# microsoft/crescent-credentials

Hardware: AMD Instinct MI355X
Metric: Groth16 proofs/sec (rs256-sd-shaped circuit, BN254), G1 MSM scalar-adds/sec reported alongside (higher is better)
Workload: dtype u32 limbs (BN254 Fq/Fr, 254-bit modular integers)

## Files before the change

### crescent-credentials_amd/csrc/csr_host.hpp

```cpp
#pragma once
#include <string.h>

#include <algorithm>
#include <unordered_map>
#include <vector>

#include "curve.hpp"
#include "errors.hpp"
#include "host_parallel.hpp"

namespace cg {

static constexpr uint32_t SELL_PIECE = 8;
static constexpr uint32_t SELL_FINAL = 0x80000000u;
static constexpr uint32_t SELL_PAD = 0xffffffffu;

struct HostSellLevel {
    uint32_t n_pieces = 0, n_partials = 0;
    std::vector<uint32_t> slice_ptr;
    RawArray<uint32_t> dst, col, cidx;
    size_t n_slots = 0;
};
struct HostCsr {
    uint64_t rows = 0, nnz = 0;
    std::vector<uint32_t> rp;
    RawArray<uint32_t> idx;
    std::vector<Fr> dict_mont;
    std::vector<uint32_t> long_rows;
    std::vector<HostSellLevel> levels;
    uint32_t sell_scratch = 0;
};

inline std::vector<uint64_t> range_bounds(uint64_t n, uint64_t min_chunk) {
    uint64_t parts = std::min<uint64_t>(host_threads(), (n + min_chunk - 1) / (min_chunk ? min_chunk : 1));
    if (parts < 1) parts = 1;
    std::vector<uint64_t> b(parts + 1);
    for (uint64_t k = 0; k <= parts; ++k) b[k] = n * k / parts;
    return b;
}
template <class Fn>
inline void for_ranges(const std::vector<uint64_t>& bounds, Fn fn) {
    const uint64_t parts = bounds.size() - 1;
    parallel_ranges(parts, 1, [&](uint64_t a, uint64_t b) { for (uint64_t k = a; k < b; ++k) fn(k, bounds[k], bounds[k + 1]); });
}

#ifdef CSR_HOST_TIMING
#include <chrono>
#include <stdio.h>
#define CSR_LAP(name) do { auto _n = std::chrono::steady_clock::now(); fprintf(stderr, "    %-28s %.1f ms\n", name, std::chrono::duration<double, std::milli>(_n - _lap).count()); _lap = _n; } while (0)
#define CSR_LAP_START auto _lap = std::chrono::steady_clock::now()
#else
#define CSR_LAP(name) do {} while (0)
#define CSR_LAP_START do {} while (0)
#endif
namespace csr_detail {
struct Key {
    uint64_t w[4];
    bool operator==(const Key& o) const { return !memcmp(w, o.w, 32); }
};
struct KeyHash {
    size_t operator()(const Key& k) const { return (size_t)(k.w[0] * 0x9e3779b97f4a7c15ull ^ k.w[1] ^ (k.w[2] << 1) ^ (k.w[3] << 7)); }
};
}

inline void csr_build_sell_host(HostCsr& out, const uint32_t* col_h, bool reorder);

inline void csr_prepare_host(const cg_csr& m, uint64_t rows, uint64_t num_variables, bool sliced, bool reorder, HostCsr& out) {
    using namespace csr_detail;
    out.rows = rows;
    out.nnz = m.nnz;
    const uint64_t nnz = m.nnz;
    if (nnz >= (1ull << 32)) throw HipError(CG_ERR_INVALID_ARGUMENT, "matrix with >= 2^32 non-zeros");
    if (m.row_ptr[0] != 0 || m.row_ptr[rows] != nnz) throw HipError(CG_ERR_INVALID_ARGUMENT, "row_ptr does not span [0, nnz]");
    CSR_LAP_START;
    out.rp.resize(rows + 1);
    parallel_ranges(rows + 1, 1u << 16, [&](uint64_t lo, uint64_t hi) {
        for (uint64_t i = lo; i < hi; ++i) {
            if (i && m.row_ptr[i] < m.row_ptr[i - 1]) throw HipError(CG_ERR_INVALID_ARGUMENT, "row_ptr not monotone");
            out.rp[i] = (uint32_t)m.row_ptr[i];
        }
    });
    CSR_LAP("row_ptr");
    out.idx.alloc(nnz);
    uint32_t* idx = out.idx.p;
    const std::vector<uint64_t> tb = range_bounds(nnz, 1u << 16);
    const uint64_t parts = tb.size() - 1;
    std::vector<std::vector<Key>> local_keys(parts);
    for (auto& v : local_keys) v.reserve(1024);
    for_ranges(tb, [&](uint64_t k, uint64_t lo, uint64_t hi) {
        std::unordered_map<Key, uint32_t, KeyHash> map;
        std::vector<Key>& keys = local_keys[k];
        Key last{};
        uint32_t last_id = 0;
        bool have_last = false;
        for (uint64_t t = lo; t < hi; ++t) {
            if (m.col[t] >= num_variables) throw HipError(CG_ERR_INVALID_ARGUMENT, "column index out of range");
            Key key;
            memcpy(key.w, m.coeff + 32 * t, 32);
            if (key.w[0] == 1 && !(key.w[1] | key.w[2] | key.w[3])) { idx[t] = 0; continue; }
            if (have_last && key == last) { idx[t] = last_id; continue; }
            auto it = map.find(key);
            if (it == map.end()) {
                it = map.emplace(key, (uint32_t)keys.size()).first;
                keys.push_back(key);
            }
            last = key; last_id = it->second | 0x80000000u; have_last = true;
            idx[t] = last_id;
        }
    });
    CSR_LAP("local dictionaries");
    std::vector<Fr> dict_h;
    {
        Fr o = Fr::zero(); o.l[0] = 1;
        dict_h.push_back(o);
    }
    constexpr uint32_t MERGE_PARTS = 16;
    std::vector<std::vector<uint32_t>> remap(parts);
    for (uint64_t k = 0; k < parts; ++k) remap[k].resize(local_keys[k].size());
    std::vector<std::vector<Key>> class_keys(MERGE_PARTS);
    std::vector<std::exception_ptr> class_err(MERGE_PARTS);
    parallel_ranges(MERGE_PARTS, 1, [&](uint64_t lo, uint64_t hi) {
        for (uint64_t cls = lo; cls < hi; ++cls) {
            std::unordered_map<Key, uint32_t, KeyHash> mine;
            std::vector<Key>& ck = class_keys[cls];
            for (uint64_t k = 0; k < parts; ++k)
                for (size_t j = 0; j < local_keys[k].size(); ++j) {
                    const Key& key = local_keys[k][j];
                    if ((KeyHash()(key) >> 7) % MERGE_PARTS != cls) continue;
                    auto it = mine.find(key);
                    if (it == mine.end()) {
                        bool lt = false;
                        for (int q = 3; q >= 0; --q) {
                            const uint64_t nq = (uint64_t)FrP::N[2 * q] | ((uint64_t)FrP::N[2 * q + 1] << 32);
                            if (key.w[q] != nq) { lt = key.w[q] < nq; break; }
                        }
                        if (!lt) throw HipError(CG_ERR_INVALID_ARGUMENT, "non-canonical matrix coefficient");
                        it = mine.emplace(key, (uint32_t)ck.size()).first;
                        ck.push_back(key);
                    }
                    remap[k][j] = it->second | ((uint32_t)cls << 27);
                }
        }
    });
    uint32_t class_off[MERGE_PARTS + 1];
    class_off[0] = 1;
    for (uint32_t cls = 0; cls < MERGE_PARTS; ++cls) {
        if (class_keys[cls].size() >= (1u << 27)) throw HipError(CG_ERR_INVALID_ARGUMENT, "too many distinct matrix coefficients");
        class_off[cls + 1] = class_off[cls] + (uint32_t)class_keys[cls].size();
    }
    dict_h.resize(class_off[MERGE_PARTS]);
    parallel_ranges(MERGE_PARTS, 1, [&](uint64_t lo, uint64_t hi) {
        for (uint64_t cls = lo; cls < hi; ++cls)
            for (size_t j = 0; j < class_keys[cls].size(); ++j) memcpy(dict_h[class_off[cls] + j].l, class_keys[cls][j].w, 32);
    });
    for (uint64_t k = 0; k < parts; ++k)
        for (uint32_t& v : remap[k]) v = class_off[v >> 27] + (v & ((1u << 27) - 1));
    CSR_LAP("merge");
    for_ranges(tb, [&](uint64_t k, uint64_t lo, uint64_t hi) {
        const uint32_t* rm = remap[k].data();
        for (uint64_t t = lo; t < hi; ++t)
            if (idx[t] & 0x80000000u) idx[t] = rm[idx[t] & 0x7fffffffu];
    });
    parallel_ranges(dict_h.size(), 1u << 12, [&](uint64_t lo, uint64_t hi) { for (uint64_t i = lo; i < hi; ++i) dict_h[i] = to_mont(dict_h[i]); });
    out.dict_mont.swap(dict_h);
    CSR_LAP("remap + to_mont");
    out.long_rows.clear();
    for (uint64_t i = 0; i < rows; ++i)
        if (out.rp[i + 1] - out.rp[i] > 4096u) out.long_rows.push_back((uint32_t)i);
    out.levels.clear();
    out.sell_scratch = 0;
    CSR_LAP("long rows");
    if (sliced) csr_build_sell_host(out, m.col, reorder);
    CSR_LAP("sliced layout");
}

inline void csr_build_sell_host(HostCsr& out, const uint32_t* col_h, bool reorder) {
    struct Item { uint32_t row, first, len; };
    struct Piece { uint32_t first, len, dst; };
    const uint64_t rows = out.rows, nnz = out.nnz;
    const std::vector<uint32_t>& rp = out.rp;
    CSR_LAP_START;
    RawArray<uint32_t> cur_col, cur_idx;
    cur_col.alloc(nnz);
    cur_idx.alloc(nnz);
    parallel_ranges(nnz, 1u << 18, [&](uint64_t lo, uint64_t hi) {
        memcpy(cur_col.p + lo, col_h + lo, (hi - lo) * 4);
        memcpy(cur_idx.p + lo, out.idx.p + lo, (hi - lo) * 4);
    });
    if (reorder)
        parallel_ranges(rows, 1u << 14, [&](uint64_t lo, uint64_t hi) {
            for (uint64_t i = lo; i < hi; ++i) {
                uint32_t w = rp[i];
                for (uint32_t t = rp[i]; t < rp[i + 1]; ++t)
                    if (cur_idx.p[t] != 0) {
                        std::swap(cur_idx.p[t], cur_idx.p[w]);
                        std::swap(cur_col.p[t], cur_col.p[w]);
                        ++w;
                    }
            }
        });
    CSR_LAP("  copy + reorder");
    RawArray<Item> items;
    size_t n_items = 0;
    {
        const std::vector<uint64_t> rb = range_bounds(rows, 1u << 14);
        std::vector<uint64_t> cnt(rb.size(), 0);
        for_ranges(rb, [&](uint64_t k, uint64_t lo, uint64_t hi) {
            uint64_t c = 0;
            for (uint64_t i = lo; i < hi; ++i) c += rp[i + 1] > rp[i];
            cnt[k + 1] = c;
        });
        for (size_t k = 1; k < cnt.size(); ++k) cnt[k] += cnt[k - 1];
        n_items = cnt.back();
        items.alloc(n_items);
        for_ranges(rb, [&](uint64_t k, uint64_t lo, uint64_t hi) {
            uint64_t at = cnt[k];
            for (uint64_t i = lo; i < hi; ++i)
                if (rp[i + 1] > rp[i]) items.p[at++] = {(uint32_t)i, rp[i], rp[i + 1] - rp[i]};
        });
    }
    CSR_LAP("  items");
    const uint32_t* ccol = cur_col.p;
    const uint32_t* cidx = cur_idx.p;
    RawArray<uint32_t> next_col_buf;
    while (n_items) {
        if (out.levels.size() >= 8) throw HipError(CG_ERR_INVALID_ARGUMENT, "matrix row too long for the sliced layout");
        out.levels.emplace_back();
        HostSellLevel& L = out.levels.back();
        const std::vector<uint64_t> ib = range_bounds(n_items, 1u << 13);
        const size_t nr = ib.size() - 1;
        std::vector<uint64_t> c_pieces(nr + 1, 0), c_next(nr + 1, 0), c_part(nr + 1, 0);
        for_ranges(ib, [&](uint64_t k, uint64_t lo, uint64_t hi) {
            uint64_t p = 0, n = 0, q = 0;
            for (uint64_t i = lo; i < hi; ++i) {
                const uint32_t np = (items.p[i].len + SELL_PIECE - 1) / SELL_PIECE;
                p += np;
                if (np > 1) { n += 1; q += np; }
            }
            c_pieces[k + 1] = p; c_next[k + 1] = n; c_part[k + 1] = q;
        });
        for (size_t k = 1; k <= nr; ++k) { c_pieces[k] += c_pieces[k - 1]; c_next[k] += c_next[k - 1]; c_part[k] += c_part[k - 1]; }
        const uint64_t n_pieces = c_pieces[nr], partials = c_part[nr];
        if (n_pieces >= (1ull << 31) || partials >= (1ull << 31)) throw HipError(CG_ERR_INVALID_ARGUMENT, "matrix too large for the sliced layout");
        RawArray<Piece> pieces, sorted;
        RawArray<Item> next_items;
        pieces.alloc(n_pieces);
        sorted.alloc(n_pieces);
        next_items.alloc(c_next[nr]);
        RawArray<uint32_t> next_col;
        next_col.alloc(partials);
        for_ranges(ib, [&](uint64_t k, uint64_t lo, uint64_t hi) {
            uint64_t p = c_pieces[k], n = c_next[k], q = c_part[k];
            for (uint64_t i = lo; i < hi; ++i) {
                const Item& it = items.p[i];
                const uint32_t np = (it.len + SELL_PIECE - 1) / SELL_PIECE;
                if (np == 1) {
                    pieces.p[p++] = {it.first, it.len, it.row | SELL_FINAL};
                    continue;
                }
                next_items.p[n++] = {it.row, (uint32_t)q, np};
                for (uint32_t j = 0; j < np; ++j) {
                    const uint32_t b = it.first + j * SELL_PIECE;
                    const uint32_t l = it.len - j * SELL_PIECE < SELL_PIECE ? it.len - j * SELL_PIECE : SELL_PIECE;
                    pieces.p[p++] = {b, l, (uint32_t)q};
                    next_col.p[q] = (uint32_t)q;
                    ++q;
                }
            }
        });
        CSR_LAP("  pieces");
        constexpr uint32_t NK = (SELL_PIECE + 1) * (SELL_PIECE + 1);
        auto key_of = [&](const Piece& p) {
            uint32_t k = 0;
            if (reorder)
                for (uint32_t t = 0; t < p.len; ++t) k += cidx[p.first + t] != 0;
            return (SELL_PIECE - k) * (SELL_PIECE + 1) + (SELL_PIECE - p.len);
        };
        const std::vector<uint64_t> pb = range_bounds(n_pieces, 1u << 13);
        const size_t npr = pb.size() - 1;
        RawArray<uint8_t> keys;
        keys.alloc(n_pieces);
        std::vector<uint64_t> hist((npr + 1) * NK, 0);
        for_ranges(pb, [&](uint64_t k, uint64_t lo, uint64_t hi) {
            uint64_t* h = &hist[k * NK];
            for (uint64_t i = lo; i < hi; ++i) { keys.p[i] = (uint8_t)key_of(pieces.p[i]); h[keys.p[i]]++; }
        });
        {
            uint64_t run = 0;
            for (uint32_t key = 0; key < NK; ++key)
                for (size_t k = 0; k < npr; ++k) { const uint64_t c = hist[k * NK + key]; hist[k * NK + key] = run; run += c; }
        }
        for_ranges(pb, [&](uint64_t k, uint64_t lo, uint64_t hi) {
            uint64_t* h = &hist[k * NK];
            for (uint64_t i = lo; i < hi; ++i) sorted.p[h[keys.p[i]]++] = pieces.p[i];
        });
        CSR_LAP("  sort");
        const uint32_t np = (uint32_t)n_pieces, ns = (np + 63) / 64;
        L.slice_ptr.assign(ns + 1, 0);
        L.dst.alloc(np ? np : 1);
        if (!np) L.dst.p[0] = 0;
        parallel_ranges(ns, 1u << 10, [&](uint64_t lo, uint64_t hi) {
            for (uint64_t s = lo; s < hi; ++s) {
                uint32_t longest = 0;
                for (uint32_t p = (uint32_t)s * 64; p < np && p < ((uint32_t)s + 1) * 64; ++p) longest = std::max(longest, sorted.p[p].len);
                L.slice_ptr[s + 1] = 64 * longest;
            }
        });
        for (uint32_t s = 0; s < ns; ++s) L.slice_ptr[s + 1] += L.slice_ptr[s];
        const size_t n_slots = L.slice_ptr[ns] ? L.slice_ptr[ns] : 1;
        L.n_slots = n_slots;
        L.col.alloc(n_slots);
        L.cidx.alloc(n_slots);
        const uint32_t* sp = L.slice_ptr.data();
        uint32_t* lc = L.col.p;
        uint32_t* li = L.cidx.p;
        if (!ns) { lc[0] = 0; li[0] = SELL_PAD; }
        parallel_ranges(ns, 1u << 8, [&](uint64_t lo, uint64_t hi) {
            for (uint64_t s = lo; s < hi; ++s) {
                for (uint32_t t = sp[s]; t < sp[s + 1]; ++t) { lc[t] = 0; li[t] = SELL_PAD; }
                for (uint32_t p = (uint32_t)s * 64; p < np && p < ((uint32_t)s + 1) * 64; ++p) {
                    const Piece& pc = sorted.p[p];
                    L.dst.p[p] = pc.dst;
                    const uint32_t base = sp[s] + (p & 63);
                    for (uint32_t t = 0; t < pc.len; ++t) {
                        lc[base + t * 64] = ccol[pc.first + t];
                        li[base + t * 64] = cidx[pc.first + t];
                    }
                }
            }
        });
        CSR_LAP("  fill");
        L.n_pieces = np;
        L.n_partials = (uint32_t)partials;
        if (L.n_partials > out.sell_scratch) out.sell_scratch = L.n_partials;
        n_items = c_next[nr];
        items = std::move(next_items);
        next_col_buf = std::move(next_col);
        ccol = next_col_buf.p;
        cur_idx.alloc(partials);
        parallel_ranges(partials, 1u << 18, [&](uint64_t lo, uint64_t hi) { memset(cur_idx.p + lo, 0, (hi - lo) * 4); });
        cidx = cur_idx.p;
    }
}

}
```

### crescent-credentials_amd/csrc/field29.hpp

```cpp
#pragma once
#include "field.hpp"

namespace cg {

static constexpr uint32_t M29 = (1u << 29) - 1u;

struct Fq29P {
    static constexpr uint32_t N[9] = {0x187cfd47u, 0x010460b6u, 0x1c72a34fu, 0x02d522d0u, 0x1585d978u,
                                      0x02db40c0u, 0x00a6e141u, 0x0e5c2634u, 0x0030644eu};
    static constexpr uint32_t NINV = 0x04866389u;
    static constexpr uint32_t ONE[9] = {0x157ccc21u, 0x141c2758u, 0x185230d3u, 0x014c0419u, 0x0aa36fb9u,
                                        0x1d4240ceu, 0x11d54c07u, 0x052ac7a8u, 0x000dc836u};
    static constexpr uint32_t R2[9] = {0x059bac10u, 0x0d1503a3u, 0x018016b8u, 0x10ab0ca8u, 0x02632639u,
                                       0x02c0169fu, 0x169bfd53u, 0x11869d4cu, 0x002a11a6u};
    static constexpr uint32_t C256[9] = {0x13349ca1u, 0x1a5d84a8u, 0x0a3e5cacu, 0x100249e0u, 0x12b951e8u,
                                         0x0e92d304u, 0x14cb95b3u, 0x041b9d3du, 0x00058003u};
    typedef FqP P256;
};
struct Fr29P {
    static constexpr uint32_t N[9] = {0x10000001u, 0x1f0fac9fu, 0x0e5c2450u, 0x07d090f3u, 0x1585d283u,
                                      0x02db40c0u, 0x00a6e141u, 0x0e5c2634u, 0x0030644eu};
    static constexpr uint32_t NINV = 0x0fffffffu;
    static constexpr uint32_t ONE[9] = {0x0fffff57u, 0x1ea70ab4u, 0x052c068bu, 0x17504f49u, 0x0aa8075bu,
                                        0x1d4240ceu, 0x11d54c07u, 0x052ac7a8u, 0x000dc836u};
// ... 103 lines not shown
#pragma unroll
        for (int i = 0; i <= k; ++i) { c += (uint64_t)a.l[i] * b.l[k - i]; CG_PIN(c); }
#pragma unroll
        for (int i = 0; i < k; ++i) { c += (uint64_t)m[i] * P::N[k - i]; CG_PIN(c); }
        m[k] = ((uint32_t)c * P::NINV) & M29;
        c += (uint64_t)m[k] * P::N[0];
        c >>= 29;
    }
#pragma unroll
    for (int k = 9; k < 17; ++k) {
#pragma unroll
        for (int i = k - 8; i <= 8; ++i) {
            c += (uint64_t)a.l[i] * b.l[k - i]; CG_PIN(c);
            c += (uint64_t)m[i] * P::N[k - i]; CG_PIN(c);
        }
        r.l[k - 9] = (uint32_t)c & M29;
        c >>= 29;
    }
    r.l[8] = (uint32_t)c;
    return r;
}
template <class P>
CG_HD F29<P> sqr_core(const F29<P>& a) {
    uint64_t c = 0;
    uint32_t m[9], d[9];
    F29<P> r;
#pragma unroll
    for (int i = 0; i < 9; ++i) d[i] = a.l[i] << 1;
#pragma unroll
    for (int k = 0; k < 9; ++k) {
#pragma unroll
        for (int i = 0; 2 * i < k; ++i) { c += (uint64_t)d[i] * a.l[k - i]; CG_PIN(c); }
        if ((k & 1) == 0) { c += (uint64_t)a.l[k / 2] * a.l[k / 2]; CG_PIN(c); }
#pragma unroll
        for (int i = 0; i < k; ++i) { c += (uint64_t)m[i] * P::N[k - i]; CG_PIN(c); }
        m[k] = ((uint32_t)c * P::NINV) & M29;
        c += (uint64_t)m[k] * P::N[0];
        c >>= 29;
    }
#pragma unroll
    for (int k = 9; k < 17; ++k) {
#pragma unroll
        for (int i = k - 8; 2 * i < k; ++i) { c += (uint64_t)d[i] * a.l[k - i]; CG_PIN(c); }
        if ((k & 1) == 0) { c += (uint64_t)a.l[k / 2] * a.l[k / 2]; CG_PIN(c); }
#pragma unroll
        for (int i = k - 8; i <= 8; ++i) { c += (uint64_t)m[i] * P::N[k - i]; CG_PIN(c); }
        r.l[k - 9] = (uint32_t)c & M29;
        c >>= 29;
    }
    r.l[8] = (uint32_t)c;
    return r;
}

template <class P>
CG_HD F29<P> mul(const F29<P>& a, const F29<P>& b) { return mul_core(a, b); }
template <class P>
CG_HD F29<P> sqr(const F29<P>& a) { return sqr_core(a); }

template <class P>
CG_HD F29<P> cond_sub_n(const F29<P>& a) {
    F29<P> t;
    uint32_t borrow = 0;
#pragma unroll
    for (int i = 0; i < 9; ++i) {
        uint32_t d = a.l[i] - P::N[i] - borrow;
        borrow = d >> 31;
        t.l[i] = (i < 8) ? (d & M29) : d;
    }
    F29<P> r;
#pragma unroll
    for (int i = 0; i < 9; ++i) r.l[i] = borrow ? a.l[i] : t.l[i];
    return r;
}

template <class P>
CG_HD F29<P> canonical(const F29<P>& a) {
    return cond_sub_n(mul(a, F29<P>::one()));
}
template <class P>
CG_HD bool is_zero_mod(const F29<P>& a) {
    uint32_t z = 0, e = 0;
#pragma unroll
    for (int i = 0; i < 9; ++i) {
        z |= a.l[i];
        e |= a.l[i] ^ P::N[i];
    }
    return z == 0 || e == 0;
}

template <class P>
CG_HD bool maybe_zero_mod(const F29<P>& a) { return a.l[0] == 0u || a.l[0] == P::N[0]; }

template <class P>
CG_HD F29<P> unpack29(const uint32_t w[8]) {
    F29<P> r;
#pragma unroll
    for (int i = 0; i < 9; ++i) {
        const int bit = 29 * i, wi = bit >> 5, sh = bit & 31;
        uint64_t v = w[wi];
        if (wi + 1 < 8) v |= (uint64_t)w[wi + 1] << 32;
        r.l[i] = (uint32_t)(v >> sh) & (i < 8 ? M29 : 0xffffffffu);
    }
    return r;
}
template <class P>
CG_HD void pack29(const F29<P>& a, uint32_t w[8]) {
#pragma unroll
    for (int j = 0; j < 8; ++j) {
        const int lo = (32 * j) / 29, sh = 32 * j - 29 * lo;
        uint64_t v = (uint64_t)a.l[lo] >> sh;
        v |= (uint64_t)a.l[lo + 1] << (29 - sh);
        if (lo + 2 < 9 && 58 - sh < 32) v |= (uint64_t)a.l[lo + 2] << (58 - sh);
        w[j] = (uint32_t)v;
    }
}

template <class P>
CG_HD F29<P> from_canonical_bytes(const Fp<typename P::P256>& c) {
    return canonical(mul(unpack29<P>(c.l), F29<P>::from_limbs(P::R2)));
}
template <class P>
CG_HD F29<P> from_mont256(const Fp<typename P::P256>& c) {
    return canonical(mul(unpack29<P>(c.l), F29<P>::from_limbs(P::C256)));
}
template <class P>
CG_HD Fp<typename P::P256> to_canonical_bytes(const F29<P>& a) {
    F29<P> one = F29<P>::zero();
    one.l[0] = 1;
    F29<P> t = cond_sub_n(mul(a, one));
    Fp<typename P::P256> r;
    pack29(t, r.l);
    return r;
}

using Fq29 = F29<Fq29P>;
using Fr29 = F29<Fr29P>;

CG_HD Fr29 weak_reduce(const Fr29& v) {
    constexpr uint32_t MU = 88753990u;
    const uint32_t q = (uint32_t)(((uint64_t)v.l[8] * MU) >> 48);
    const int32_t nq = -(int32_t)q;
    Fr29 r;
    int64_t c = 0;
#pragma unroll
    for (int i = 0; i < 9; ++i) {
        c += (int64_t)v.l[i];
        c += (int64_t)nq * (int64_t)(int32_t)Fr29P::N[i];
        if (i < 8) { r.l[i] = (uint32_t)c & M29; c >>= 29; }
        else r.l[i] = (uint32_t)c;
    }
    return r;
}

CG_HD void bfly(Fr29& u, Fr29& v, const Fr29& w) {
    Fr29 t = mul(v, w);
    v = sub<3, 1>(u, t);
    u = add(u, t);
}

template <class P>
struct S29 {
    int32_t l[9];
    CG_HD static S29 from_unsigned(const F29<P>& a) {
        S29 r;
#pragma unroll
        for (int i = 0; i < 9; ++i) r.l[i] = (int32_t)a.l[i];
        return r;
    }
    CG_HD static S29 one() { return from_unsigned(F29<P>::one()); }
};
struct NoFuse { CG_HD void operator()(int, int64_t&) const {} };
template <class P>
struct FuseMul1 {
    const S29<P>& x; int32_t s;
    CG_HD void operator()(int j, int64_t& c) const { c += (int64_t)x.l[j] * (int64_t)s; }
};
template <class P>
struct FuseMul2 {
    const S29<P>& x; int32_t s1; const S29<P>& y; int32_t s2;
    CG_HD void operator()(int j, int64_t& c) const { c += (int64_t)x.l[j] * (int64_t)s1; CG_PIN(c); c += (int64_t)y.l[j] * (int64_t)s2; }
};
#define CG_SN(i) ((int64_t)(int32_t)P::N[i])
template <class P, class Fuse>
CG_HD S29<P> mul_s(const S29<P>& a, const S29<P>& b, Fuse fuse) {
    int64_t c = 0;
    int32_t m[9];
    S29<P> r;
#pragma unroll
    for (int k = 0; k < 9; ++k) {
#pragma unroll
        for (int i = 0; i <= k; ++i) { c += (int64_t)a.l[i] * (int64_t)b.l[k - i]; CG_PIN(c); }
#pragma unroll
        for (int i = 0; i < k; ++i) { c += (int64_t)m[i] * CG_SN(k - i); CG_PIN(c); }
        m[k] = (int32_t)(((uint32_t)c * P::NINV) & M29);
        c += (int64_t)m[k] * CG_SN(0);
        c >>= 29;
    }
#pragma unroll
    for (int k = 9; k < 17; ++k) {
#pragma unroll
        for (int i = k - 8; i <= 8; ++i) {
            c += (int64_t)a.l[i] * (int64_t)b.l[k - i]; CG_PIN(c);
            c += (int64_t)m[i] * CG_SN(k - i); CG_PIN(c);
        }
        fuse(k - 9, c); CG_PIN(c);
        r.l[k - 9] = (int32_t)((uint32_t)c & M29);
        c >>= 29;
    }
    fuse(8, c);
    r.l[8] = (int32_t)c;
    return r;
}
template <class P>
CG_HD S29<P> mul_s(const S29<P>& a, const S29<P>& b) { return mul_s(a, b, NoFuse{}); }
template <class P, class Fuse>
CG_HD S29<P> sqr_s(const S29<P>& a, Fuse fuse) {
    int64_t c = 0;
    int32_t m[9], d[9];
    S29<P> r;
#pragma unroll
    for (int i = 0; i < 9; ++i) d[i] = a.l[i] * 2;
#pragma unroll
    for (int k = 0; k < 9; ++k) {
#pragma unroll
        for (int i = 0; 2 * i < k; ++i) { c += (int64_t)d[i] * (int64_t)a.l[k - i]; CG_PIN(c); }
        if ((k & 1) == 0) { c += (int64_t)a.l[k / 2] * (int64_t)a.l[k / 2]; CG_PIN(c); }
#pragma unroll
        for (int i = 0; i < k; ++i) { c += (int64_t)m[i] * CG_SN(k - i); CG_PIN(c); }
        m[k] = (int32_t)(((uint32_t)c * P::NINV) & M29);
        c += (int64_t)m[k] * CG_SN(0);
        c >>= 29;
    }
#pragma unroll
    for (int k = 9; k < 17; ++k) {
#pragma unroll
        for (int i = k - 8; 2 * i < k; ++i) { c += (int64_t)d[i] * (int64_t)a.l[k - i]; CG_PIN(c); }
        if ((k & 1) == 0) { c += (int64_t)a.l[k / 2] * (int64_t)a.l[k / 2]; CG_PIN(c); }
#pragma unroll
        for (int i = k - 8; i <= 8; ++i) { c += (int64_t)m[i] * CG_SN(k - i); CG_PIN(c); }
        fuse(k - 9, c); CG_PIN(c);
        r.l[k - 9] = (int32_t)((uint32_t)c & M29);
        c >>= 29;
    }
    fuse(8, c);
    r.l[8] = (int32_t)c;
    return r;
}
template <class P>
CG_HD S29<P> sqr_s(const S29<P>& a) { return sqr_s(a, NoFuse{}); }
template <class P>
CG_HD S29<P> mul2_s(const S29<P>& x0, const S29<P>& y0, const S29<P>& x1, const S29<P>& y1) {
    int64_t c = 0;
    int32_t m[9];
    S29<P> r;
#pragma unroll
    for (int k = 0; k < 9; ++k) {
#pragma unroll
        for (int i = 0; i <= k; ++i) {
            c += (int64_t)x0.l[i] * (int64_t)y0.l[k - i]; CG_PIN(c);
            c += (int64_t)x1.l[i] * (int64_t)y1.l[k - i]; CG_PIN(c);
        }
#pragma unroll
        for (int i = 0; i < k; ++i) { c += (int64_t)m[i] * CG_SN(k - i); CG_PIN(c); }
        m[k] = (int32_t)(((uint32_t)c * P::NINV) & M29);
        c += (int64_t)m[k] * CG_SN(0);
        c >>= 29;
    }
#pragma unroll
    for (int k = 9; k < 17; ++k) {
#pragma unroll
        for (int i = k - 8; i <= 8; ++i) {
            c += (int64_t)x0.l[i] * (int64_t)y0.l[k - i]; CG_PIN(c);
            c += (int64_t)x1.l[i] * (int64_t)y1.l[k - i]; CG_PIN(c);
            c += (int64_t)m[i] * CG_SN(k - i); CG_PIN(c);
        }
        r.l[k - 9] = (int32_t)((uint32_t)c & M29);
        c >>= 29;
    }
    r.l[8] = (int32_t)c;
    return r;
}
#undef CG_SN
template <int K, class P>
CG_HD F29<P> to_unsigned(const S29<P>& a) {
    F29<P> r;
    int32_t c = 0;
#pragma unroll
    for (int i = 0; i < 8; ++i) {
        const int32_t t = a.l[i] + (int32_t)KN<P, K, 0>::value.v[i] + c;
        r.l[i] = (uint32_t)t & M29;
        c = t >> 29;
    }
    r.l[8] = (uint32_t)(a.l[8] + (int32_t)KN<P, K, 0>::value.v[8] + c);
    return r;
}
template <class P>
CG_HD bool is_zero_mod(const S29<P>& a) {
    uint32_t z = 0, e = 0;
#pragma unroll
    for (int i = 0; i < 9; ++i) {
        z |= (uint32_t)a.l[i];
        e |= (uint32_t)a.l[i] ^ P::N[i];
    }
    return z == 0 || e == 0;
}
using Fq29s = S29<Fq29P>;
// ... 105 lines not shown
```

### crescent-credentials_amd/csrc/wmap29.hip

```cpp
#include "wmap29.hpp"
#include "satcheck.hpp"

namespace cg {

static constexpr int TS29_SMALL = 10, TS29_BIG = 11;
static int strided_max_stages(int tile_log) { return tile_log == TS29_BIG ? 10 : 6; }
static int ntt_passes(int logn, int tile_log) {
    if (logn <= tile_log) return 1;
    const int smax = strided_max_stages(tile_log);
    return 1 + (logn - tile_log + smax - 1) / smax;
}
static int ntt_tile_log(int logn) {
    static const int forced = [] {
        const char* e = CG_TUNE_ENV("NTT_TILE");
        return (e && (atoi(e) == TS29_SMALL || atoi(e) == TS29_BIG)) ? atoi(e) : 0;
    }();
    if (forced) return (forced == TS29_BIG && logn > TS29_SMALL) ? TS29_BIG : TS29_SMALL;
    return (logn >= 20 && ntt_passes(logn, TS29_BIG) < ntt_passes(logn, TS29_SMALL)) ? TS29_BIG : TS29_SMALL;
}

__device__ __forceinline__ Fr29 load_packed29(const uint32_t* __restrict__ base, uint64_t idx) {
    const uint4* p = reinterpret_cast<const uint4*>(base + idx * 8);
    uint4 a = p[0], b = p[1];
    uint32_t w[8] = {a.x, a.y, a.z, a.w, b.x, b.y, b.z, b.w};
    return unpack29<Fr29P>(w);
}
__device__ __forceinline__ void store_packed29(uint32_t* __restrict__ base, uint64_t idx, const Fr29& canonical_value) {
    uint32_t w[8];
    pack29(canonical_value, w);
    uint4* p = reinterpret_cast<uint4*>(base + idx * 8);
    p[0] = make_uint4(w[0], w[1], w[2], w[3]);
    p[1] = make_uint4(w[4], w[5], w[6], w[7]);
}
__device__ __forceinline__ uint32_t brev(uint32_t x, int bits) { return bits ? (__brev(x) >> (32 - bits)) : 0u; }

__global__ void __launch_bounds__(256) k_to_packed29(const Fr* __restrict__ in, uint32_t* __restrict__ out, uint64_t n, int plain,
                                                     int unbitrev_logn) {
    uint64_t i = (uint64_t)blockIdx.x * blockDim.x + threadIdx.x;
    if (i >= n) return;
    Fr x = in[i];
    uint64_t dst = unbitrev_logn ? brev((uint32_t)i, unbitrev_logn) : i;
    if (plain) {
        Fr c = from_mont(x);
        uint4* p = reinterpret_cast<uint4*>(out + dst * 8);
        p[0] = make_uint4(c.l[0], c.l[1], c.l[2], c.l[3]);
        p[1] = make_uint4(c.l[4], c.l[5], c.l[6], c.l[7]);
    } else {
        store_packed29(out, dst, from_mont256<Fr29P>(x));
    }
}

__global__ void __launch_bounds__(256) k_to_limbs12(const Fr* __restrict__ in, uint32_t* __restrict__ out, uint64_t n) {
    uint64_t i = (uint64_t)blockIdx.x * blockDim.x + threadIdx.x;
    if (i >= n) return;
    Fr29 x = from_mont256<Fr29P>(in[i]);
    uint4* p = reinterpret_cast<uint4*>(out + i * 12);
    p[0] = make_uint4(x.l[0], x.l[1], x.l[2], x.l[3]);
    p[1] = make_uint4(x.l[4], x.l[5], x.l[6], x.l[7]);
    p[2] = make_uint4(x.l[8], 0u, 0u, 0u);
}
__device__ __forceinline__ Fr29 load_tw(const uint32_t* __restrict__ tw, uint64_t idx) {
    const uint4* p = reinterpret_cast<const uint4*>(tw + idx * 12);
    uint4 a = p[0], b = p[1], c = p[2];
    Fr29 r;
    r.l[0] = a.x; r.l[1] = a.y; r.l[2] = a.z; r.l[3] = a.w;
    r.l[4] = b.x; r.l[5] = b.y; r.l[6] = b.z; r.l[7] = b.w;
    r.l[8] = c.x;
    return r;
}

void Wm29Domain::build(const NttDomain& d, hipStream_t st) {
    logn = d.logn;
    n = d.n;
    const uint64_t half = n > 1 ? n / 2 : 1;
    tw_fwd.alloc(half * 12);
    tw_inv.alloc(half * 12);
    coset.alloc(n * 8);
    icoset.alloc(n * 8);
    k_to_limbs12<<<ceil_div(half, 256), 256, 0, st>>>(d.tw_fwd.p, tw_fwd.p, half);
    k_to_limbs12<<<ceil_div(half, 256), 256, 0, st>>>(d.tw_inv.p, tw_inv.p, half);
    if (d.coset_br.n) {
        k_to_packed29<<<ceil_div(n, 256), 256, 0, st>>>(d.coset_br.p, coset.p, n, 0, logn);
        k_to_packed29<<<ceil_div(n, 256), 256, 0, st>>>(d.icoset_br.p, icoset.p, n, 1, logn);
    }
    CG_KERNEL_CHECK();
    Fr29 v = from_mont256<Fr29P>(d.vanishing_inv);
    pack29(v, vinv);
    Fr vp = from_mont(d.vanishing_inv);
    memcpy(vinv_plain, vp.l, 32);
}

void Wm29Strided::build(const NttDomain& big, int logs_, int rank, hipStream_t st) {
    logs = logs_;
    d = big.n >> logs;
    NttDomain small;
    small.build(big.logn - logs, false, st);
    sub.build(small, st);
    const Fr s = mul(fr_from_u64(5), fr_pow_u64(fr_root_of_unity(big.logn), (uint64_t)rank));
    DevBuf<Fr> t(big.n);
    fr_pow_table(t.p, s, inv(fr_from_u64(big.n)), big.n, false, big.logn, st);
    fold.alloc(big.n * 8);
    k_to_packed29<<<ceil_div(big.n, 256), 256, 0, st>>>(t.p, fold.p, big.n, 0, 0);
    CG_KERNEL_CHECK();
    CG_HIP(hipStreamSynchronize(st));
}

__global__ void __launch_bounds__(256) k_fold29(const uint32_t* __restrict__ a, const uint32_t* __restrict__ T, uint32_t* __restrict__ out,
                                                uint32_t d, int logd, uint32_t terms) {
    const uint32_t i = blockIdx.x * blockDim.x + threadIdx.x;
    if (i >= d) return;
    Fr29 acc = Fr29::zero();
    for (uint32_t t = 0; t < terms; ++t) {
        const uint64_t e = (uint64_t)i + (uint64_t)t * d;
        acc = add(acc, mul(load_packed29(a, e), load_packed29(T, e)));
        if ((t & 3u) == 3u) acc = normalize(acc);
        if ((t & 63u) == 63u) acc = weak_reduce(acc);
    }
    store_packed29(out, brev(i, logd), weak_reduce(normalize(acc)));
}

void Csr29::build(const DevCsr& m, hipStream_t st) {
    dict.alloc(m.dict.n * 8);
    k_to_packed29<<<ceil_div(m.dict.n, 256), 256, 0, st>>>(m.dict.p, dict.p, m.dict.n, 0, 0);
    CG_KERNEL_CHECK();
}

__device__ __forceinline__ bool fr_lt_modulus(const Fr& x) {
    bool lt = false, decided = false;
#pragma unroll
    for (int k = 7; k >= 0; --k) {
        if (!decided && x.l[k] != FrP::N[k]) { lt = x.l[k] < FrP::N[k]; decided = true; }
    }
    return lt;
}

__global__ void __launch_bounds__(256) k_w_to29(const Fr* __restrict__ w, uint32_t* __restrict__ out, uint64_t n,
                                                uint32_t* __restrict__ bad_input, uint32_t* __restrict__ va, uint64_t m, uint64_t l, int logn) {
    uint64_t i = (uint64_t)blockIdx.x * blockDim.x + threadIdx.x;
    if (i >= n) return;
    Fr x = w[i];
    if (!fr_lt_modulus(x)) *bad_input = 1u;
    const Fr29 v = mul(unpack29<Fr29P>(x.l), Fr29::from_limbs(Fr29P::R2));
    store_packed29(out, i, v);
    if (i < l) store_packed29(va, brev((uint32_t)(m + i), logn), v);
}


__global__ void __launch_bounds__(256) k_sell29(const uint32_t* __restrict__ slice_ptr, const uint32_t* __restrict__ col,
                                                const uint32_t* __restrict__ cidx, const uint32_t* __restrict__ dst,
                                                const uint32_t* __restrict__ dict, const uint32_t* __restrict__ src,
                                                uint32_t* __restrict__ out, uint32_t* __restrict__ scratch, uint32_t n_pieces, int logn) {
    const uint32_t p = blockIdx.x * blockDim.x + threadIdx.x;
    if (p >= n_pieces) return;
    const uint32_t s = p >> 6, lane = p & 63u;
    const uint32_t base = slice_ptr[s], len = (slice_ptr[s + 1] - base) >> 6;
    Fr29 acc = Fr29::zero();
    uint32_t cnt = 0;
#if !defined(CG_SELL_BATCH)
#define CG_SELL_BATCH 0
#endif
#if CG_SELL_BATCH == 0
    for (uint32_t t = 0; t < len; ++t) {
        const uint32_t ci = cidx[base + t * 64 + lane];
        if (ci == SELL_PAD) continue;
        Fr29 v = load_packed29(src, col[base + t * 64 + lane]);
        if (ci != 0) v = mul(v, load_packed29(dict, ci));
        acc = add(acc, v);
        if ((++cnt & 3u) == 0) acc = normalize(acc);
    }
#else
    constexpr uint32_t BS = CG_SELL_BATCH;
    uint32_t ci[SELL_PIECE], cl[SELL_PIECE];
#pragma unroll
    for (uint32_t t = 0; t < SELL_PIECE; ++t) {
        const bool in = t < len;
        ci[t] = in ? cidx[base + t * 64 + lane] : SELL_PAD;
        cl[t] = in ? col[base + t * 64 + lane] : 0u;
    }
#pragma unroll
    for (uint32_t h = 0; h < SELL_PIECE; h += BS) {
        if (h >= len) break;
        uint4 rv[BS][2], rd[BS][2];
#pragma unroll
        for (uint32_t u = 0; u < BS; ++u) {
            const uint32_t t = h + u;
            if (ci[t] == SELL_PAD) continue;
            const uint4* pv = reinterpret_cast<const uint4*>(src + (uint64_t)cl[t] * 8);
            rv[u][0] = pv[0]; rv[u][1] = pv[1];
            if (ci[t] != 0) {
                const uint4* pd = reinterpret_cast<const uint4*>(dict + (uint64_t)ci[t] * 8);
                rd[u][0] = pd[0]; rd[u][1] = pd[1];
            }
        }
#pragma unroll
        for (uint32_t u = 0; u < BS; ++u) {
            const uint32_t t = h + u;
            if (ci[t] == SELL_PAD) continue;
            const uint32_t wv[8] = {rv[u][0].x, rv[u][0].y, rv[u][0].z, rv[u][0].w, rv[u][1].x, rv[u][1].y, rv[u][1].z, rv[u][1].w};
            Fr29 v = unpack29<Fr29P>(wv);
            if (ci[t] != 0) {
                const uint32_t wd[8] = {rd[u][0].x, rd[u][0].y, rd[u][0].z, rd[u][0].w, rd[u][1].x, rd[u][1].y, rd[u][1].z, rd[u][1].w};
                v = mul(v, unpack29<Fr29P>(wd));
            }
            acc = add(acc, v);
            if ((++cnt & 3u) == 0) acc = normalize(acc);
        }
    }
#endif
    const uint32_t d = dst[p];
    const Fr29 r = weak_reduce(normalize(acc));
    if (d & SELL_FINAL) store_packed29(out, brev(d & ~SELL_FINAL, logn), r);
    else store_packed29(scratch, d, r);
}

struct Pass29 {
    int logn, ts, S, cbits, gbit_lo, q0;
};
__device__ __forceinline__ uint32_t l2g29(uint32_t e, uint32_t tile, const Pass29& pp) {
    const int extra_bits = pp.ts - pp.S - pp.cbits;
    uint32_t colv = e & ((1u << pp.cbits) - 1u);
    uint32_t g = (e >> pp.cbits) & ((1u << pp.S) - 1u);
    uint32_t extra = e >> (pp.cbits + pp.S);
    uint32_t T = (tile << extra_bits) | extra;
    const int lo_bits = pp.gbit_lo - pp.cbits;
    uint32_t Tlo = T & ((1u << lo_bits) - 1u);
    uint32_t Thi = T >> lo_bits;
    return colv | (Tlo << pp.cbits) | (g << pp.gbit_lo) | (Thi << (pp.gbit_lo + pp.S));
}
__device__ __forceinline__ uint32_t lds_off(uint32_t e) { return e * 9u + (e >> 5); }
__device__ __forceinline__ Fr29 lds_get(const uint32_t* s, uint32_t e) {
    Fr29 r;
    const uint32_t o = lds_off(e);
#pragma unroll
    for (int i = 0; i < 9; ++i) r.l[i] = s[o + i];
    return r;
}
__device__ __forceinline__ void lds_put(uint32_t* s, uint32_t e, const Fr29& x) {
    const uint32_t o = lds_off(e);
#pragma unroll
    for (int i = 0; i < 9; ++i) s[o + i] = x.l[i];
}

struct Packed8 { uint32_t w[8]; };

template <int LOAD, int STORE, int TSL>
__global__ void __launch_bounds__(256 << (TSL - 10)) k_ntt29_pass(const uint32_t* __restrict__ in_a, const uint32_t* __restrict__ in_b,
                                                    const uint32_t* __restrict__ in_c, uint32_t* __restrict__ out,
                                                    const uint32_t* __restrict__ tw, const uint32_t* __restrict__ scale,
                                                    Packed8 vinv_p, Pass29 pp, int store_bitrev) {
    __shared__ uint32_t sm[(1 << TSL) * 9 + (1 << TSL) / 16];
    constexpr uint32_t NT = 256u << (TSL - 10);
    const uint32_t tile = blockIdx.x;
    const uint32_t tsize = 1u << pp.ts;
    for (uint32_t e = threadIdx.x; e < tsize; e += NT) {
        uint32_t gi = l2g29(e, tile, pp);
        Fr29 x = load_packed29(in_a, gi);
        if (LOAD == 1) {
            Fr29 bb = load_packed29(in_b, gi), cc = load_packed29(in_c, gi);
            Fr29 vinv = unpack29<Fr29P>(vinv_p.w);
            x = mul(normalize(sub<7, 1>(mul(x, bb), cc)), vinv);
        }
        lds_put(sm, e, x);
    }
    auto group_of = [&](int jj, uint32_t& k, int& sh1, int& sh2) {
        const int q = pp.q0 + jj;
        const int lb = pp.cbits + (q - pp.gbit_lo);
        const uint32_t lmask = (1u << lb) - 1u;
        sh1 = pp.logn - 1 - q; sh2 = pp.logn - 2 - q;
        const uint32_t bb = threadIdx.x;
        const uint32_t e00 = ((bb & ~lmask) << 2) | (bb & lmask);
        k = l2g29(e00, tile, pp) & ((1u << q) - 1u);
    };
    auto first_twiddle_of = [&](int jj, Fr29& w) {
        if (jj + 1 >= pp.S || threadIdx.x >= (tsize >> 2)) return;
        uint32_t k; int sh1, sh2;
        group_of(jj, k, sh1, sh2);
        w = (pp.q0 + jj == 0) ? load_tw(tw, (uint64_t)1 << sh2) : load_tw(tw, (uint64_t)k << sh1);
    };
    Fr29 w_first;
    first_twiddle_of(0, w_first);
    __syncthreads();
    int j = 0;
    for (; j + 1 < pp.S; j += 2) {
        const int q = pp.q0 + j;
        const int lb = pp.cbits + (q - pp.gbit_lo);
        const uint32_t lmask = (1u << lb) - 1u;
        const int sh2 = pp.logn - 2 - q;
        for (uint32_t b = threadIdx.x; b < (tsize >> 2); b += NT) {
            const uint32_t e00 = ((b & ~lmask) << 2) | (b & lmask);
            const uint32_t e01 = e00 | (1u << lb), e10 = e00 | (2u << lb), e11 = e00 | (3u << lb);
            const uint32_t gi = l2g29(e00, tile, pp);
            const uint32_t k = gi & ((1u << q) - 1u);
            Fr29 x0 = lds_get(sm, e00), x1 = lds_get(sm, e01), x2 = lds_get(sm, e10), x3 = lds_get(sm, e11);
            if (q == 0) {
                Fr29 t = x1;
                x1 = sub<7, 1>(x0, t);
                x0 = add(x0, t);
                t = x3;
                x3 = sub<7, 1>(x2, t);
                x2 = add(x2, t);
                t = x2;
                x2 = sub<12, 2>(x0, t);
                x0 = add(x0, t);
                bfly(x1, x3, w_first);
            } else {
                const Fr29 w2a = load_tw(tw, (uint64_t)k << sh2);
                const Fr29 w2b = load_tw(tw, (uint64_t)(k + (1u << q)) << sh2);
                bfly(x0, x1, w_first);
                bfly(x2, x3, w_first);
                bfly(x0, x2, w2a);
                bfly(x1, x3, w2b);
            }
            lds_put(sm, e00, normalize(x0));
            lds_put(sm, e01, normalize(x1));
            lds_put(sm, e10, normalize(x2));
            lds_put(sm, e11, normalize(x3));
        }
        first_twiddle_of(j + 2, w_first);
#if defined(CG_NTT_WAVE_LOCAL)
        const int lb_next = lb + 2;
        const bool wave_local = (j + 3 < pp.S) && ((4u << lb_next) <= 256u) && (tsize >> 2) >= 64u;
        if (wave_local) __builtin_amdgcn_fence(__ATOMIC_ACQ_REL, "wavefront");
        else __syncthreads();
#else
        __syncthreads();
#endif
    }
    if (j < pp.S) {
        const int q = pp.q0 + j;
        const int lb = pp.cbits + (q - pp.gbit_lo);
        const uint32_t lmask = (1u << lb) - 1u;
        const int tw_shift = pp.logn - 1 - q;
        for (uint32_t b = threadIdx.x; b < (tsize >> 1); b += NT) {
            uint32_t e0 = ((b & ~lmask) << 1) | (b & lmask);
            uint32_t e1 = e0 | (1u << lb);
            uint32_t gi = l2g29(e0, tile, pp);
            uint32_t k = gi & ((1u << q) - 1u);
            Fr29 u = lds_get(sm, e0), v = lds_get(sm, e1);
            bfly(u, v, load_tw(tw, (uint64_t)k << tw_shift));
            lds_put(sm, e0, normalize(u));
            lds_put(sm, e1, normalize(v));
        }
        __syncthreads();
    }
    const uint32_t smask = (1u << pp.S) - 1u;
    for (uint32_t f = threadIdx.x; f < tsize; f += NT) {
        uint32_t e = f;
        if (store_bitrev) {
            uint32_t gprime = f & smask, colp = f >> pp.S;
            e = (brev(gprime, pp.S) << pp.cbits) | colp;
        }
        uint32_t gi = l2g29(e, tile, pp);
        Fr29 x = lds_get(sm, e);
        Fr29 y;
        if (STORE == 1) y = cond_sub_n(mul(x, load_packed29(scale, gi)));
        else if (STORE == 2) y = cond_sub_n(mul(x, unpack29<Fr29P>(vinv_p.w)));
        else if (STORE == 3) y = cond_sub_n(mul(load_packed29(in_b, gi), x));
        else y = weak_reduce(x);
        store_packed29(out, store_bitrev ? brev(gi, pp.logn) : gi, y);
    }
}
// ... 243 lines not shown
```

Baseline: 185.0.

## Specialize SELL sparse matvec terms for power-of-two and minus-one coefficients

On the host, each matrix coefficient is classified as ±2^k, ±1, or general. Rows and pieces are sorted by class, and the cidx entries are tagged so the SELL kernel can split each slice into regions. In those regions the kernel uses a cheap shift-and-reduce multiply or a plain add/negate instead of loading a dictionary entry and doing a full Montgomery multiply. This cuts dictionary loads and multiplies for the sparse R1CS matrix-vector step, at the cost of a wave-ballot pre-pass in the kernel, more complex host preprocessing, and removal of the batched-load variant.

```diff
diff --git a/crescent-credentials_amd/csrc/csr_host.hpp b/crescent-credentials_amd/csrc/csr_host.hpp
--- a/crescent-credentials_amd/csrc/csr_host.hpp
+++ b/crescent-credentials_amd/csrc/csr_host.hpp
@@ -15,9 +15,43 @@
 static constexpr uint32_t SELL_FINAL = 0x80000000u;
 static constexpr uint32_t SELL_PAD = 0xffffffffu;
 
+static constexpr uint32_t SELL_TAG_SHIFT = 0x40000000u;
+static constexpr uint32_t SELL_TAG_MINUS = 0x80000000u;
+static constexpr uint32_t SELL_TAG_MASK = 0xc0000000u;
+static constexpr uint32_t SELL_NEG = 0x100u;
+static constexpr uint32_t SELL_MINUS_ONE = SELL_TAG_MINUS | SELL_NEG;
+static constexpr uint32_t SELL_SHIFT_MAX = 30;
+static constexpr uint32_t SELL_NO_CODE = 0xfffffffeu;
+CG_HD uint32_t sell_class(uint32_t code) { return code == SELL_NO_CODE ? 3u : (code & 0xffu) ? 2u : code ? 1u : 0u; }
+CG_HD uint32_t sell_regions_pack(uint32_t prod, uint32_t shift, uint32_t minus) { return prod | (shift << 4) | (minus << 8); }
+CG_HD uint32_t sell_region_prod(uint32_t r) { return r & 15u; }
+CG_HD uint32_t sell_region_shift(uint32_t r) { return (r >> 4) & 15u; }
+CG_HD uint32_t sell_region_minus(uint32_t r) { return (r >> 8) & 15u; }
+
+inline uint32_t sell_code_of(const uint64_t w[4]) {
+    auto pow2 = [](const uint64_t x[4]) -> uint32_t {
+        if (x[1] | x[2] | x[3]) return SELL_NO_CODE;
+        for (uint32_t k = 0; k <= SELL_SHIFT_MAX; ++k)
+            if (x[0] == (1ull << k)) return k;
+        return SELL_NO_CODE;
+    };
+    uint32_t k = pow2(w);
+    if (k != SELL_NO_CODE) return k;
+    uint64_t neg[4], borrow = 0;
+    for (int q = 0; q < 4; ++q) {
+        const uint64_t nq = (uint64_t)FrP::N[2 * q] | ((uint64_t)FrP::N[2 * q + 1] << 32);
+        const uint64_t d = nq - w[q];
+        neg[q] = d - borrow;
+        borrow = (nq < w[q]) | (d < borrow);
+    }
+    k = pow2(neg);
+    return k == SELL_NO_CODE ? SELL_NO_CODE : (k | SELL_NEG);
+}
+
 struct HostSellLevel {
     uint32_t n_pieces = 0, n_partials = 0;
     std::vector<uint32_t> slice_ptr;
+    std::vector<uint32_t> regions;
     RawArray<uint32_t> dst, col, cidx;
     size_t n_slots = 0;
 };
@@ -26,6 +60,7 @@
     std::vector<uint32_t> rp;
     RawArray<uint32_t> idx;
     std::vector<Fr> dict_mont;
+    std::vector<uint32_t> sell_code;
     std::vector<uint32_t> long_rows;
     std::vector<HostSellLevel> levels;
     uint32_t sell_scratch = 0;
@@ -148,6 +183,7 @@
         if (class_keys[cls].size() >= (1u << 27)) throw HipError(CG_ERR_INVALID_ARGUMENT, "too many distinct matrix coefficients");
         class_off[cls + 1] = class_off[cls] + (uint32_t)class_keys[cls].size();
     }
+    if (class_off[MERGE_PARTS] >= SELL_TAG_SHIFT) throw HipError(CG_ERR_INVALID_ARGUMENT, "too many distinct matrix coefficients");
     dict_h.resize(class_off[MERGE_PARTS]);
     parallel_ranges(MERGE_PARTS, 1, [&](uint64_t lo, uint64_t hi) {
         for (uint64_t cls = lo; cls < hi; ++cls)
@@ -161,7 +197,15 @@
         for (uint64_t t = lo; t < hi; ++t)
             if (idx[t] & 0x80000000u) idx[t] = rm[idx[t] & 0x7fffffffu];
     });
-    parallel_ranges(dict_h.size(), 1u << 12, [&](uint64_t lo, uint64_t hi) { for (uint64_t i = lo; i < hi; ++i) dict_h[i] = to_mont(dict_h[i]); });
+    out.sell_code.resize(dict_h.size());
+    parallel_ranges(dict_h.size(), 1u << 12, [&](uint64_t lo, uint64_t hi) {
+        for (uint64_t i = lo; i < hi; ++i) {
+            uint64_t cw[4];
+            memcpy(cw, dict_h[i].l, 32);
+            out.sell_code[i] = sell_code_of(cw);
+            dict_h[i] = to_mont(dict_h[i]);
+        }
+    });
     out.dict_mont.swap(dict_h);
     CSR_LAP("remap + to_mont");
     out.long_rows.clear();
@@ -187,16 +231,29 @@
         memcpy(cur_col.p + lo, col_h + lo, (hi - lo) * 4);
         memcpy(cur_idx.p + lo, out.idx.p + lo, (hi - lo) * 4);
     });
+    const uint32_t* code = out.sell_code.data();
     if (reorder)
         parallel_ranges(rows, 1u << 14, [&](uint64_t lo, uint64_t hi) {
+            std::vector<uint32_t> tc, ti;
             for (uint64_t i = lo; i < hi; ++i) {
-                uint32_t w = rp[i];
-                for (uint32_t t = rp[i]; t < rp[i + 1]; ++t)
-                    if (cur_idx.p[t] != 0) {
-                        std::swap(cur_idx.p[t], cur_idx.p[w]);
-                        std::swap(cur_col.p[t], cur_col.p[w]);
-                        ++w;
-                    }
+                const uint32_t b = rp[i], n = rp[i + 1] - rp[i];
+                uint32_t cnt[4] = {0, 0, 0, 0};
+                bool sorted = true;
+                for (uint32_t t = 0; t < n; ++t) {
+                    const uint32_t c = sell_class(code[cur_idx.p[b + t]]);
+                    if (t && c > sell_class(code[cur_idx.p[b + t - 1]])) sorted = false;
+                    cnt[c]++;
+                }
+                if (sorted) continue;
+                uint32_t at[4];
+                at[3] = 0; at[2] = cnt[3]; at[1] = at[2] + cnt[2]; at[0] = at[1] + cnt[1];
+                tc.resize(n); ti.resize(n);
+                for (uint32_t t = 0; t < n; ++t) {
+                    const uint32_t w = at[sell_class(code[cur_idx.p[b + t]])]++;
+                    tc[w] = cur_col.p[b + t]; ti[w] = cur_idx.p[b + t];
+                }
+                memcpy(cur_col.p + b, tc.data(), (size_t)n * 4);
+                memcpy(cur_idx.p + b, ti.data(), (size_t)n * 4);
             }
         });
     CSR_LAP("  copy + reorder");
@@ -269,21 +326,22 @@
             }
         });
         CSR_LAP("  pieces");
-        constexpr uint32_t NK = (SELL_PIECE + 1) * (SELL_PIECE + 1);
+        constexpr uint32_t K1 = SELL_PIECE + 1, NK = K1 * K1 * K1 * K1;
         auto key_of = [&](const Piece& p) {
-            uint32_t k = 0;
+            uint32_t n[4] = {0, 0, 0, 0};
             if (reorder)
-                for (uint32_t t = 0; t < p.len; ++t) k += cidx[p.first + t] != 0;
-            return (SELL_PIECE - k) * (SELL_PIECE + 1) + (SELL_PIECE - p.len);
+                for (uint32_t t = 0; t < p.len; ++t) n[sell_class(code[cidx[p.first + t]])]++;
+            const uint32_t k = n[1] + n[2] + n[3];
+            return (((SELL_PIECE - k) * K1 + (SELL_PIECE - p.len)) * K1 + (SELL_PIECE - n[3])) * K1 + (SELL_PIECE - n[2]);
         };
         const std::vector<uint64_t> pb = range_bounds(n_pieces, 1u << 13);
         const size_t npr = pb.size() - 1;
-        RawArray<uint8_t> keys;
+        RawArray<uint16_t> keys;
         keys.alloc(n_pieces);
         std::vector<uint64_t> hist((npr + 1) * NK, 0);
         for_ranges(pb, [&](uint64_t k, uint64_t lo, uint64_t hi) {
             uint64_t* h = &hist[k * NK];
-            for (uint64_t i = lo; i < hi; ++i) { keys.p[i] = (uint8_t)key_of(pieces.p[i]); h[keys.p[i]]++; }
+            for (uint64_t i = lo; i < hi; ++i) { keys.p[i] = (uint16_t)key_of(pieces.p[i]); h[keys.p[i]]++; }
         });
         {
             uint64_t run = 0;
@@ -315,16 +373,28 @@
         uint32_t* lc = L.col.p;
         uint32_t* li = L.cidx.p;
         if (!ns) { lc[0] = 0; li[0] = SELL_PAD; }
+        L.regions.assign(ns ? ns : 1, 0);
+        uint32_t* rg = L.regions.data();
         parallel_ranges(ns, 1u << 8, [&](uint64_t lo, uint64_t hi) {
             for (uint64_t s = lo; s < hi; ++s) {
                 for (uint32_t t = sp[s]; t < sp[s + 1]; ++t) { lc[t] = 0; li[t] = SELL_PAD; }
+                uint32_t cls[SELL_PIECE];
+                for (uint32_t t = 0; t < SELL_PIECE; ++t) cls[t] = 0;
+                for (uint32_t p = (uint32_t)s * 64; p < np && p < ((uint32_t)s + 1) * 64; ++p) {
+                    const Piece& pc = sorted.p[p];
+                    for (uint32_t t = 0; t < pc.len; ++t) cls[t] = std::max(cls[t], reorder ? sell_class(code[cidx[pc.first + t]]) : 3u);
+                }
+                uint32_t n_of[4] = {0, 0, 0, 0};
+                for (uint32_t t = 0; t < (sp[s + 1] - sp[s]) / 64; ++t) n_of[cls[t]]++;
+                rg[s] = sell_regions_pack(n_of[3], n_of[3] + n_of[2], n_of[3] + n_of[2] + n_of[1]);
                 for (uint32_t p = (uint32_t)s * 64; p < np && p < ((uint32_t)s + 1) * 64; ++p) {
                     const Piece& pc = sorted.p[p];
                     L.dst.p[p] = pc.dst;
                     const uint32_t base = sp[s] + (p & 63);
                     for (uint32_t t = 0; t < pc.len; ++t) {
+                        const uint32_t ix = cidx[pc.first + t];
                         lc[base + t * 64] = ccol[pc.first + t];
-                        li[base + t * 64] = cidx[pc.first + t];
+                        li[base + t * 64] = cls[t] == 3 ? ix : cls[t] == 2 ? (SELL_TAG_SHIFT | code[ix]) : cls[t] == 1 ? (SELL_TAG_MINUS | code[ix]) : 0u;
                     }
                 }
             }
diff --git a/crescent-credentials_amd/csrc/field29.hpp b/crescent-credentials_amd/csrc/field29.hpp
--- a/crescent-credentials_amd/csrc/field29.hpp
+++ b/crescent-credentials_amd/csrc/field29.hpp
@@ -279,6 +279,28 @@
     return r;
 }
 
+CG_HD Fr29 mul_pow2(const Fr29& v, uint32_t k, bool negative) {
+    constexpr uint32_t MU2 = 2840127684u;
+    const uint32_t t = (v.l[8] << 8) | (v.l[7] >> 21);
+    uint64_t q = ((uint64_t)t * MU2) >> (61u - k);
+    if (negative) q += 5u;
+    const int32_t s = negative ? -1 : 1;
+    const int32_t m = s * (int32_t)(1u << k);
+    const int32_t q0 = -s * (int32_t)((uint32_t)q & M29), q1 = -s * (int32_t)(uint32_t)(q >> 29);
+    Fr29 r;
+    int64_t c = 0;
+#pragma unroll
+    for (int i = 0; i < 9; ++i) {
+        c += (int64_t)(int32_t)v.l[i] * (int64_t)m;
+        c += (int64_t)q0 * (int64_t)(int32_t)Fr29P::N[i];
+        if (i) c += (int64_t)q1 * (int64_t)(int32_t)Fr29P::N[i - 1];
+        r.l[i] = (uint32_t)c & M29;
+        c >>= 29;
+    }
+    return r;
+}
+CG_HD Fr29 neg_packed(const Fr29& v) { return sub<7, 1>(Fr29::zero(), v); }
+
 CG_HD void bfly(Fr29& u, Fr29& v, const Fr29& w) {
     Fr29 t = mul(v, w);
     v = sub<3, 1>(u, t);
diff --git a/crescent-credentials_amd/csrc/wmap29.hip b/crescent-credentials_amd/csrc/wmap29.hip
--- a/crescent-credentials_amd/csrc/wmap29.hip
+++ b/crescent-credentials_amd/csrc/wmap29.hip
@@ -153,60 +153,56 @@
     const uint32_t p = blockIdx.x * blockDim.x + threadIdx.x;
     if (p >= n_pieces) return;
     const uint32_t s = p >> 6, lane = p & 63u;
-    const uint32_t base = slice_ptr[s], len = (slice_ptr[s + 1] - base) >> 6;
+    const uint32_t base = (uint32_t)__builtin_amdgcn_readfirstlane((int)slice_ptr[s]);
+    const uint32_t len = ((uint32_t)__builtin_amdgcn_readfirstlane((int)slice_ptr[s + 1]) - base) >> 6;
+    const uint32_t* ci_at = cidx + base + lane;
+    const uint32_t* col_at = col + base + lane;
+    uint32_t e_prod = 0, e_shift = 0, e_minus = 0;
+    for (uint32_t t = 0; t < len; ++t) {
+        const uint32_t ci = ci_at[t * 64];
+        const bool term = ci != SELL_PAD;
+        const uint32_t tag = ci & SELL_TAG_MASK;
+        const bool product = __ballot(term && tag == 0u && ci != 0u) != 0ull;
+        const bool shift = __ballot(term && tag == SELL_TAG_SHIFT) != 0ull;
+        const bool minus = __ballot(term && tag == SELL_TAG_MINUS) != 0ull;
+        e_prod += product;
+        e_shift += product || shift;
+        e_minus += product || shift || minus;
+    }
     Fr29 acc = Fr29::zero();
-    uint32_t cnt = 0;
-#if !defined(CG_SELL_BATCH)
-#define CG_SELL_BATCH 0
-#endif
-#if CG_SELL_BATCH == 0
-    for (uint32_t t = 0; t < len; ++t) {
-        const uint32_t ci = cidx[base + t * 64 + lane];
+    uint32_t weight = 0;
+#define SELL_ROOM(w) do { if (weight + (w) > 4u) { acc = normalize(acc); weight = 0; } weight += (w); } while (0)
+    uint32_t t = 0;
+    for (; t < e_prod; ++t) {
+        SELL_ROOM(1u);
+        const uint32_t ci = ci_at[t * 64];
         if (ci == SELL_PAD) continue;
-        Fr29 v = load_packed29(src, col[base + t * 64 + lane]);
+        Fr29 v = load_packed29(src, col_at[t * 64]);
         if (ci != 0) v = mul(v, load_packed29(dict, ci));
         acc = add(acc, v);
-        if ((++cnt & 3u) == 0) acc = normalize(acc);
-    }
-#else
-    constexpr uint32_t BS = CG_SELL_BATCH;
-    uint32_t ci[SELL_PIECE], cl[SELL_PIECE];
+    }
+    for (; t < e_shift; ++t) {
+        SELL_ROOM(1u);
+        const uint32_t ci = ci_at[t * 64];
+        if (ci == SELL_PAD) continue;
+        acc = add(acc, mul_pow2(load_packed29(src, col_at[t * 64]), ci & 0xffu, (ci & SELL_NEG) != 0));
+    }
+    for (; t < e_minus; ++t) {
+        SELL_ROOM(2u);
+        const uint32_t ci = ci_at[t * 64];
+        if (ci == SELL_PAD) continue;
+        const Fr29 v = load_packed29(src, col_at[t * 64]);
+        const Fr29 nv = neg_packed(v);
 #pragma unroll
-    for (uint32_t t = 0; t < SELL_PIECE; ++t) {
-        const bool in = t < len;
-        ci[t] = in ? cidx[base + t * 64 + lane] : SELL_PAD;
-        cl[t] = in ? col[base + t * 64 + lane] : 0u;
-    }
-#pragma unroll
-    for (uint32_t h = 0; h < SELL_PIECE; h += BS) {
-        if (h >= len) break;
-        uint4 rv[BS][2], rd[BS][2];
-#pragma unroll
-        for (uint32_t u = 0; u < BS; ++u) {
-            const uint32_t t = h + u;
-            if (ci[t] == SELL_PAD) continue;
-            const uint4* pv = reinterpret_cast<const uint4*>(src + (uint64_t)cl[t] * 8);
-            rv[u][0] = pv[0]; rv[u][1] = pv[1];
-            if (ci[t] != 0) {
-                const uint4* pd = reinterpret_cast<const uint4*>(dict + (uint64_t)ci[t] * 8);
-                rd[u][0] = pd[0]; rd[u][1] = pd[1];
-            }
-        }
-#pragma unroll
-        for (uint32_t u = 0; u < BS; ++u) {
-            const uint32_t t = h + u;
-            if (ci[t] == SELL_PAD) continue;
-            const uint32_t wv[8] = {rv[u][0].x, rv[u][0].y, rv[u][0].z, rv[u][0].w, rv[u][1].x, rv[u][1].y, rv[u][1].z, rv[u][1].w};
-            Fr29 v = unpack29<Fr29P>(wv);
-            if (ci[t] != 0) {
-                const uint32_t wd[8] = {rd[u][0].x, rd[u][0].y, rd[u][0].z, rd[u][0].w, rd[u][1].x, rd[u][1].y, rd[u][1].z, rd[u][1].w};
-                v = mul(v, unpack29<Fr29P>(wd));
-            }
-            acc = add(acc, v);
-            if ((++cnt & 3u) == 0) acc = normalize(acc);
-        }
-    }
-#endif
+        for (int i = 0; i < 9; ++i) acc.l[i] += (ci & SELL_NEG) ? nv.l[i] : v.l[i];
+    }
+    for (; t < len; ++t) {
+        SELL_ROOM(1u);
+        const uint32_t ci = ci_at[t * 64];
+        if (ci == SELL_PAD) continue;
+        acc = add(acc, load_packed29(src, col_at[t * 64]));
+    }
+#undef SELL_ROOM
     const uint32_t d = dst[p];
     const Fr29 r = weak_reduce(normalize(acc));
     if (d & SELL_FINAL) store_packed29(out, brev(d & ~SELL_FINAL, logn), r);
```

Result: slower. 176.4 (-4.6%).
